# huggingface/parler-tts

Hardware: NVIDIA H100
Metric: audio codec tokens/sec (all codebooks) (higher is better)
Workload: dtype bf16

## Files before the change

### parler_tts_b200/csrc/api.cu

```cuda
#include <cstdarg>
#include <cstdlib>
#include <cstring>
#include <new>
#include <vector>

#include "common.cuh"
#include "dac.h"
#include "kernels.h"
#include "layout.h"
#include "step.h"

namespace ptts {
static thread_local std::string g_err;
void set_error(const std::string& m) { g_err = m; }
int fail(int code, const char* fmt, ...) {
  char buf[1024];
  va_list ap;
  va_start(ap, fmt);
  vsnprintf(buf, sizeof(buf), fmt, ap);
  va_end(ap);
  g_err = buf;
  return code;
}
static bool env_flag(const char* name, bool dflt) {
// ... 4 lines not shown
}

using namespace ptts;

enum DecodePath {
  DECODE_MULTI_KERNEL = 0,
  DECODE_STEP = 1,
  DECODE_CLUSTER = 2,
};

struct ProbeWindow {
  void* self_attn; void* cross_attn; void* hidden;
  int first_step, n_steps;
  int64_t self_ld, self_step, cross_step, hidden_step;
};

struct AlignWindow {
  const int32_t* heads; int n_heads;
  std::vector<int> layer_heads;
  int key0, key_len;
  float* out;
  int first_row, n_rows;
};

struct ptts_session {
  ptts_decoder_config cfg;
  DecoderLayout L;
  WorkspaceLayout W;
  const char* blob;
  char* ws;
  int sm_count;
  bool has_prompt_mask, has_enc_mask, begun, prefilled;
  ptts_gen_params gen;
  int n0;
  bool ragged;
  int sampled;
  bool decoded;
  bool slots;
  cudaStream_t cap_stream;
  cudaGraphExec_t exec;
  bool graph_ready;
  int64_t launches;
  long long* prof;
  DecodePath path;
  StepParams sp;
  ptts_sampling_ext ext;
  ptts_logits_ext lext;
  SampleOut out;
  ProbeWindow probe;
  AlignWindow align;
  int64_t graph_launches;
};

static const ptts_sampling_ext kExtOff = {0, 0.f, 1.f, 0.f, 0.f};
static const ptts_sampling_ext* active_ext(const ptts_session* s) {
  const ptts_sampling_ext& x = s->ext;
  const bool warp = s->gen.do_sample && (x.min_p > 0.f || x.typical_p < 1.f || x.epsilon_cutoff > 0.f || x.eta_cutoff > 0.f);
  return (x.no_repeat_ngram_size > 0 || warp) ? &s->ext : nullptr;
}
static const ptts_logits_ext* active_lext(const ptts_session* s) {
  const ptts_logits_ext& x = s->lext;
  const bool on = x.bias1 != nullptr || x.n_seq > 0 || x.forced_bos_token_id >= 0 || x.forced_eos_token_id >= 0 ||
                  x.remove_invalid_values || x.decay != nullptr || x.suppress != nullptr || x.begin_suppress != nullptr ||
                  x.renormalize_logits;
  return on ? &s->lext : nullptr;
}
static const SampleOut* active_out(const ptts_session* s) {
  return (s->out.logits != nullptr || s->out.scores != nullptr) ? &s->out : nullptr;
}
static const ProbeWindow* active_probe(const ptts_session* s) {
  const ProbeWindow& w = s->probe;
  return (w.self_attn != nullptr || w.cross_attn != nullptr || w.hidden != nullptr) ? &w : nullptr;
}
static const AlignWindow* active_align(const ptts_session* s) { return s->align.out != nullptr ? &s->align : nullptr; }
static DecodePath decode_path(const ptts_session* s) {
  return (active_probe(s) != nullptr || active_align(s) != nullptr) ? DECODE_MULTI_KERNEL : s->path;
}

static const ptts_sampling_ext* sampler_ext(const ptts_session* s) {
  const ptts_sampling_ext* x = active_ext(s);
  return (x == nullptr && (active_out(s) != nullptr || active_lext(s) != nullptr || s->slots)) ? &kExtOff : x;
}
static const int* slot_keys(const ptts_session* s) { return s->slots ? (const int*)(s->ws + s->W.row_key) : nullptr; }

extern "C" {

const char* ptts_last_error(void) { return g_err.c_str(); }
int ptts_version(void) { return 100; }

int ptts_decoder_blob_bytes(const ptts_decoder_config* cfg, int64_t* out_bytes) {
  PTTS_REQUIRE(cfg && out_bytes, "null argument");
  if (int e = validate_config(*cfg)) return e;
  *out_bytes = make_layout(*cfg).total;
  return PTTS_OK;
}

int ptts_decoder_pack(const ptts_decoder_config* cfg, void* blob, int32_t tensor_id, int32_t index, const void* src,
                      int32_t src_dtype, int64_t rows, int64_t cols, void* stream) {
  PTTS_REQUIRE(cfg && blob && src, "null argument");
  if (int e = validate_config(*cfg)) return e;
  PTTS_REQUIRE(src_dtype == PTTS_BF16 || src_dtype == PTTS_F32, "pack: src dtype must be bf16 or f32");
  const DecoderLayout L = make_layout(*cfg);
  cudaStream_t st = (cudaStream_t)stream;
  char* base = (char*)blob;
  MatSlot ms;
  const bool per_layer = (tensor_id >= PTTS_T_LN1_W && tensor_id <= PTTS_T_FC2);
  if (per_layer) PTTS_REQUIRE(index >= 0 && index < L.L, "pack: layer %d out of range", index);
  if (matrix_slot(L, tensor_id, index, &ms)) {
    if (tensor_id == PTTS_T_LM_HEAD) PTTS_REQUIRE(index >= 0 && index < L.K, "pack: codebook %d out of range", index);
    PTTS_REQUIRE(cols == ms.m.K, "pack: tensor %d expects %d columns, got %lld", tensor_id, ms.m.K, (long long)cols);
    PTTS_REQUIRE(rows > 0 && ms.row_off + rows <= ms.m.N, "pack: tensor %d rows %lld do not fit fused matrix of %d rows", tensor_id, (long long)rows, ms.m.N);
    return pack_matrix(src, src_dtype, rows, cols, ms.row_off, ms.m.K, base + ms.m.w, cfg->dtype, st);
  }
  const int H = L.H;
  switch (tensor_id) {
    case PTTS_T_EMBED_TOKENS:
      PTTS_REQUIRE(index >= 0 && index < L.K && rows == L.V + 1 && cols == H, "pack: embed_tokens shape");
      return pack_plain(src, src_dtype, rows * cols, base + L.embed + (int64_t)index * (L.V + 1) * H * L.es, cfg->dtype, st);
    case PTTS_T_POS_TABLE:
      PTTS_REQUIRE(!cfg->rope && rows == cfg->max_positions && cols == H, "pack: pos table shape");
      return pack_plain(src, src_dtype, rows * cols, base + L.pos, cfg->dtype, st);
    case PTTS_T_ROPE_COS:
    case PTTS_T_ROPE_SIN:
      PTTS_REQUIRE(cfg->rope && rows == cfg->max_positions && cols == PTTS_HEAD_DIM, "pack: rope table shape");
      return pack_plain(src, src_dtype, rows * cols, base + (tensor_id == PTTS_T_ROPE_COS ? L.rope_cos : L.rope_sin), cfg->dtype, st);
    case PTTS_T_LN1_W: case PTTS_T_LN1_B: case PTTS_T_LN2_W: case PTTS_T_LN2_B: case PTTS_T_LN3_W: case PTTS_T_LN3_B:
    case PTTS_T_FINAL_LN_W: case PTTS_T_FINAL_LN_B: {
      PTTS_REQUIRE(rows * cols == H, "pack: LayerNorm parameter must have %d elements", H);
      const int m = tensor_id <= PTTS_T_LN1_B ? MAT_QKV : tensor_id <= PTTS_T_LN2_B ? MAT_Q_CROSS : tensor_id <= PTTS_T_LN3_B ? MAT_FC1 : MAT_HEADS;
      const DecoderMatrix dm = decoder_matrix(L, m, index);
      const bool gamma = tensor_id == PTTS_T_LN1_W || tensor_id == PTTS_T_LN2_W || tensor_id == PTTS_T_LN3_W || tensor_id == PTTS_T_FINAL_LN_W;
      return pack_plain(src, src_dtype, H, base + (gamma ? dm.ln_w : dm.ln_b), PTTS_F32, st);
    }
    default:
      return fail(PTTS_EINVAL, "pack: unknown tensor id %d", tensor_id);
  }
}

int ptts_decoder_finalize(const ptts_decoder_config* cfg, void* blob, void* stream) {
  PTTS_REQUIRE(cfg && blob, "null argument");
  if (int e = validate_config(*cfg)) return e;
  if (cfg->dtype != PTTS_BF16) return PTTS_OK;
  const DecoderLayout L = make_layout(*cfg);
  cudaStream_t st = (cudaStream_t)stream;
  char* b = (char*)blob;
  for (int m = 0; m < MAT_COUNT; m++)
    for (int i = 0; i < (m == MAT_HEADS ? 1 : L.L); i++) {
      const DecoderMatrix d = decoder_matrix(L, m, i);
      if (d.ln_w >= 0) {
        float* c = (float*)(b + d.c);
        if (int e = fold_layernorm(b + d.w, d.N, d.K, (const float*)(b + d.ln_w), (const float*)(b + d.ln_b), c, c + d.N, st)) return e;
      }
      if (d.rm >= 0)
        if (int e = unpack_fragments(b + d.w, b + d.rm, d.N, d.K, st)) return e;
    }
  if (L.cl_NC > 0) {
    for (int i = 0; i < L.L; i++)
      if (int e = cluster_pack_layer(L, b + L.layer0 + L.layer_stride * i, st)) return e;
  }
  return PTTS_OK;
}

int ptts_workspace_bytes3(const ptts_decoder_config* cfg, int32_t B, int32_t P, int32_t S, int32_t max_cache_len, int32_t max_input_len,
                          int32_t takes, int64_t* out_bytes) {
  PTTS_REQUIRE(cfg && out_bytes, "null argument");
  if (int e = validate_config(*cfg)) return e;
// ... 501 lines not shown
  const WorkspaceLayout& W = s->W;
  PTTS_REQUIRE(T >= 1 && T <= W.max_input, "score: %d decoder input columns, the session takes 1 .. %d", T, W.max_input);
  PTTS_REQUIRE(W.P == 0 || prompt_hidden, "score: prompt_hidden is required when P > 0");
  PTTS_REQUIRE(labels ? (out_token_nll != nullptr) : (out_logits != nullptr && out_codebook_sums == nullptr),
               "score: labels need out_token_nll; without labels only out_logits can be filled");
  const bool fused = (c.dtype == PTTS_BF16 && out_logits == nullptr);
  PTTS_REQUIRE(!fused || heads_rm, "score: the fused bf16 path needs the row-major heads (ptts_lm_heads_rowmajor_pack)");
  PTTS_REQUIRE(!fused || score_fused_supported(L.H, L.V), "score: hidden_size %d / vocab_size %d are outside the fused kernel", L.H, L.V);
  cudaStream_t st = (cudaStream_t)stream;
  PTTS_CHECK_CUDA(cudaMemcpy2DAsync(s->ws + W.raw_ids, W.raw_ld * 8, dec_ids, (size_t)T * 8, (size_t)T * 8, W.BK, cudaMemcpyDeviceToDevice, st));
  s->has_prompt_mask = (prompt_mask != nullptr && W.P > 0);
  s->has_enc_mask = (enc_mask != nullptr);
  if (s->has_prompt_mask) { if (int e = launch_mask_convert(prompt_mask, W.B * W.P, (int*)(s->ws + W.prompt_mask), st)) return e; }
  if (s->has_enc_mask) { if (int e = launch_mask_convert(enc_mask, W.B / W.takes * W.S, (int*)(s->ws + W.enc_mask), st)) return e; }
  s->n0 = T;
  s->ragged = s->slots = false;
  s->begun = s->prefilled = false;
  if (int e = run_forward(s, st, true, prompt_hidden, enc_hidden, false)) return e;

  ScoreArgs a{};
  a.labels = labels; a.dec_ids = dec_ids; a.token_nll = out_token_nll;
  a.M = W.B * T; a.B = W.B; a.T = T; a.K = L.K; a.V = L.V; a.H = L.H;
  a.bos = c.bos_token_id; a.eos = c.eos_token_id;
  const int q_len = W.P + T;
  const DecoderMatrix hm = decoder_matrix(L, MAT_HEADS, 0);
  if (fused) {
    a.c1 = (const float*)(s->blob + hm.c); a.c2 = a.c1 + hm.N;
    s->launches += 2;
    if (int e = launch_score_fused(a, s->ws + W.x, W.P, c.layer_norm_eps, s->ws + W.qc, (float*)(s->ws + W.row_stats), heads_rm, st)) return e;
  } else {
    for (int t = 0; t < T; t++) {
      LinearArgs h{};
      h.X = s->ws + W.x + (int64_t)(W.P + t) * L.H * L.es; h.ldx = (int64_t)q_len * L.H;
      h.W = s->blob + hm.w; h.Y = s->ws + W.logits; h.ldy = hm.N; h.ldr = h.ldy;
      h.ln_w = (const float*)(s->blob + hm.ln_w); h.ln_b = (const float*)(s->blob + hm.ln_b); h.eps = c.layer_norm_eps;
      if (c.dtype == PTTS_BF16) { h.c1 = (const float*)(s->blob + hm.c); h.c2 = h.c1 + hm.N; }
      h.M = W.B; h.N = hm.N; h.K = hm.K; h.Kc = hm.K;
      h.epi = EPI_F32; h.act = c.activation;
      if (int e = launch_linear(h, c.dtype, st, false, s->sm_count)) return e;
      if (int e = launch_score_rows(a, (const float*)(s->ws + W.logits), t, out_logits, st)) return e;
      s->launches += 2;
    }
  }
  if (out_codebook_sums != nullptr) {
    s->launches++;
    if (int e = launch_score_reduce(a, out_codebook_sums, st)) return e;
  }
  return PTTS_OK;
}

int ptts_decode_forward(ptts_session* s, void* stream) {
  PTTS_REQUIRE(s, "null argument");
  if (!s->prefilled) return fail(PTTS_ESTATE, "ptts_decode_forward called before ptts_prefill");
  cudaStream_t st = (cudaStream_t)stream;
  s->decoded = true;
  StepParams p = s->sp;
  p.do_sample_phase = 0;
  switch (decode_path(s)) {
    case DECODE_CLUSTER: s->launches++; return launch_decode_step_cluster(p, st);
    case DECODE_STEP: s->launches++; return launch_decode_step(p, s->sm_count, st);
    case DECODE_MULTI_KERNEL: break;
  }
  return run_forward(s, st, false, nullptr, nullptr);
}

int ptts_sample(ptts_session* s, const int64_t* forced_tokens, void* stream) {
  PTTS_REQUIRE(s, "null argument");
  if (!s->prefilled) return fail(PTTS_ESTATE, "ptts_sample called before ptts_prefill");
  s->launches++;
  s->sampled++;
  return launch_sample(sample_args(s), forced_tokens, (cudaStream_t)stream, false, sampler_ext(s), active_out(s), active_lext(s),
                       slot_keys(s));
}

int ptts_decode_steps(ptts_session* s, int32_t n_steps, void* stream) {
  PTTS_REQUIRE(s && n_steps >= 0, "bad argument");
  if (!s->prefilled) return fail(PTTS_ESTATE, "ptts_decode_steps called before ptts_prefill");
  cudaStream_t st = (cudaStream_t)stream;
  if (n_steps > 0) s->decoded = true;
  const ptts_sampling_ext* ext = sampler_ext(s);
  const SampleOut* out = active_out(s);
  const ptts_logits_ext* lext = active_lext(s);
  const DecodePath path = decode_path(s);
  if (ext != nullptr && path != DECODE_MULTI_KERNEL) {
    StepParams p = s->sp;
    p.do_sample_phase = 0;
    for (int i = 0; i < n_steps; i++) {
      const int e = path == DECODE_CLUSTER ? launch_decode_step_cluster(p, st) : launch_decode_step(p, s->sm_count, st);
      if (e) return e;
      if (int e2 = launch_sample(sample_args(s), nullptr, st, false, ext, out, lext, slot_keys(s))) return e2;
    }
    s->launches += 2 * (int64_t)n_steps;
    return PTTS_OK;
  }
  switch (path) {
    case DECODE_CLUSTER: {
      const char* env = getenv("PTTS_STEPS_PER_LAUNCH");
      const int per_launch = env ? (atoi(env) < 1 ? 1 : atoi(env)) : 64;
      for (int done = 0; done < n_steps;) {
        const int m = (n_steps - done < per_launch) ? n_steps - done : per_launch;
        s->sp.n_steps = m;
        const int e = launch_decode_step_cluster(s->sp, st);
        s->sp.n_steps = 1;
        if (e) return e;
        done += m;
        s->launches += 1;
      }
      return PTTS_OK;
    }
    case DECODE_STEP:
      for (int i = 0; i < n_steps; i++)
        if (int e = launch_decode_step(s->sp, s->sm_count, st)) return e;
      s->launches += n_steps;
      return PTTS_OK;
    case DECODE_MULTI_KERNEL: break;
  }
  if (!s->graph_ready) {
    if (!s->cap_stream) PTTS_CHECK_CUDA(cudaStreamCreateWithFlags(&s->cap_stream, cudaStreamNonBlocking));
    const int64_t before = s->launches;
    PTTS_CHECK_CUDA(cudaStreamBeginCapture(s->cap_stream, cudaStreamCaptureModeThreadLocal));
    int e = run_forward(s, s->cap_stream, false, nullptr, nullptr);
    if (!e) { s->launches++; e = launch_sample(sample_args(s), nullptr, s->cap_stream, true, ext, out, lext, slot_keys(s)); }
    cudaGraph_t graph = nullptr;
    cudaError_t ce = cudaStreamEndCapture(s->cap_stream, &graph);
    s->graph_launches = s->launches - before;
    s->launches = before;
    if (e) { if (graph) cudaGraphDestroy(graph); return e; }
    if (ce != cudaSuccess) return fail(PTTS_ECUDA, "graph capture failed: %s", cudaGetErrorString(ce));
    ce = cudaGraphInstantiate(&s->exec, graph, 0);
    cudaGraphDestroy(graph);
    if (ce != cudaSuccess) return fail(PTTS_ECUDA, "graph instantiate failed: %s", cudaGetErrorString(ce));
    s->graph_ready = true;
  }
  for (int i = 0; i < n_steps; i++) PTTS_CHECK_CUDA(cudaGraphLaunch(s->exec, st));
  s->launches += s->graph_launches * n_steps;
  return PTTS_OK;
}

int ptts_session_import_rows(ptts_session* dst, const ptts_session* src, const int32_t* src_rows, const int32_t* dst_rows, int32_t n,
                             void* stream) {
  PTTS_REQUIRE(dst && src && (n == 0 || (src_rows && dst_rows)) && n >= 0, "bad argument");
  if (!src->prefilled || !dst->prefilled) return fail(PTTS_ESTATE, "import_rows: both sessions must have run ptts_prefill");
  PTTS_REQUIRE(dst != src, "import_rows: the source and the destination are one session");
  PTTS_REQUIRE(memcmp(&src->cfg, &dst->cfg, sizeof(src->cfg)) == 0 && src->blob == dst->blob, "import_rows: the sessions run different models");
  PTTS_REQUIRE(src->W.P == dst->W.P && src->W.S == dst->W.S, "import_rows: P and S must match (source %d, %d; destination %d, %d)",
               src->W.P, src->W.S, dst->W.P, dst->W.S);
  PTTS_REQUIRE(src->W.takes == 1 && dst->W.takes == 1, "import_rows: sessions with takes > 1 share cross K/V between rows");
  PTTS_REQUIRE(src->has_prompt_mask == dst->has_prompt_mask && src->has_enc_mask == dst->has_enc_mask,
               "import_rows: both sessions must have been prefilled with the same masks given (or both without)");
  PTTS_REQUIRE(!src->ragged && src->n0 == 1, "import_rows: the source rows must start from the BOS column (a uniform generation)");
  PTTS_REQUIRE(src->sampled == 1 && !src->decoded, "import_rows: the source must have run ptts_prefill and exactly one ptts_sample "
               "since (%d samples%s)", src->sampled, src->decoded ? " and decode steps" : "");
  const int kv_len = src->W.P + src->n0;
  PTTS_REQUIRE(kv_len <= dst->W.Tmax, "import_rows: %d cache positions do not fit the destination's %d", kv_len, dst->W.Tmax);
  RowImportArgs a{};
  RowRegion tmp[kMaxRowRegions];
  a.n_regions = row_regions(src->cfg, src->W, kv_len, a.src);
  PTTS_REQUIRE(row_regions(dst->cfg, dst->W, kv_len, tmp) == a.n_regions, "import_rows: the sessions hold different per-row state "
               "(create both with the same max_input_len class: 1, or >= 2)");
  for (int r = 0; r < a.n_regions; r++) a.dst[r] = tmp[r];
  a.src_ws = src->ws; a.dst_ws = dst->ws; a.K = src->cfg.num_codebooks;
  a.src_ctrl = (const Ctrl*)(src->ws + src->W.ctrl); a.dst_ctrl = (const Ctrl*)(dst->ws + dst->W.ctrl);
  std::vector<char> taken(dst->W.B, 0);
  for (int i = 0; i < n; i++) {
    PTTS_REQUIRE(src_rows[i] >= 0 && src_rows[i] < src->W.B, "import_rows: source row %d outside [0, %d)", src_rows[i], src->W.B);
    PTTS_REQUIRE(dst_rows[i] >= 0 && dst_rows[i] < dst->W.B, "import_rows: destination row %d outside [0, %d)", dst_rows[i], dst->W.B);
    PTTS_REQUIRE(!taken[dst_rows[i]], "import_rows: destination row %d is listed twice", dst_rows[i]);
    taken[dst_rows[i]] = 1;
  }
  for (int i0 = 0; i0 < n; i0 += kMaxImportRows) {
    const int m = n - i0 < kMaxImportRows ? n - i0 : kMaxImportRows;
    for (int i = 0; i < m; i++) { a.src_row[i] = src_rows[i0 + i]; a.dst_row[i] = dst_rows[i0 + i]; }
    if (int e = launch_import_rows(a, m, (cudaStream_t)stream)) return e;
// ... 297 lines not shown
```

### parler_tts_b200/csrc/step.h

```cpp
#pragma once
#include "common.cuh"
#include "kernels.h"
#include "layout.h"

namespace ptts {

struct StepParams {
  int B, H, F, V, K, L, nh, nkv, nckv, S, P, Tmax, rope, act, qkv_rows, ckv_rows;
  int takes;
  float eps, scale;
  const char* blob;
  DecoderLayout lay;
  bf16 *x, *qkv, *attn, *qc, *hbuf;
  float* logits;
  char* cross_kv; int64_t cross_layer_stride;
  char* self_kv; int64_t self_layer_stride;
  const int* prompt_mask;
  const int* enc_mask;
  SampleArgs sa;
  unsigned* bar;
  int nt_qkv, nt_h, nt_fc1, nt_heads;
  int nbuf;
  int64_t tile_region_bytes;
  int64_t wbuf_offset;
  int do_sample_phase;
  int sample_items;
  int* progress;
  int n_steps;
  long long* prof;
  bf16 *cl_x, *cl_attn, *cl_h;
};

const char* plan_decode_step(StepParams& p, int grid);
int launch_decode_step(const StepParams& p, int grid, cudaStream_t st);
bool cluster_step_available(const StepParams& p);
int launch_decode_step_cluster(const StepParams& p, cudaStream_t st);
int cluster_pack_layer(const DecoderLayout& L, char* layer, cudaStream_t st);

}
```

### parler_tts_b200/csrc/step2.cu

```cuda
#include "attn_core.cuh"
#include "common.cuh"
#include "kernels.h"
#include "ln_stats.cuh"
#include "sample_core.cuh"
#include "ptx.cuh"
#include "step.h"
#include "step_common.cuh"
#include <type_traits>

namespace ptts {
namespace cl {

constexpr int C = 2;
constexpr int V = 8;
constexpr int THREADS = 256;
constexpr int ROWS = 32;
constexpr int HROWS = 8;
constexpr int ATT_SMEM = attn_decode_smem_per_warp<bf16>();
constexpr int PROF_STRIDE = 16;
constexpr int QMAX = 6;
constexpr int OFF_STATS = 256, OFF_PART = 512, OFF_RES = 2560, OFF_CVEC = 3584;
constexpr int HDR = 5632;
constexpr int WB_BYTES = 65536;
constexpr int R_OFF = HDR + 2 * WB_BYTES;
// ... 25 lines not shown
  asm volatile("st.async.shared::cluster.mbarrier::complete_tx::bytes.b32 [%0], %1, [%2];"
               ::"r"(dst_cluster_addr), "r"(__float_as_uint(v)), "r"(bar_cluster_addr) : "memory");
}
__device__ __forceinline__ void st_async(uint32_t dst_cluster_addr, float2 v, uint32_t bar_cluster_addr) {
  asm volatile("st.async.shared::cluster.mbarrier::complete_tx::bytes.v2.f32 [%0], {%1, %2}, [%3];"
               ::"r"(dst_cluster_addr), "f"(v.x), "f"(v.y), "r"(bar_cluster_addr) : "memory");
}
__device__ __forceinline__ uint32_t mapa(uint32_t addr, uint32_t rank) { uint32_t r; asm volatile("mapa.shared::cluster.u32 %0, %1, %2;" : "=r"(r) : "r"(addr), "r"(rank)); return r; }
__device__ __forceinline__ uint32_t cluster_rank() { uint32_t r; asm volatile("mov.u32 %0, %%cluster_ctarank;" : "=r"(r)); return r; }
__device__ __forceinline__ void cluster_arrive() { asm volatile("barrier.cluster.arrive.release.aligned;" ::: "memory"); }
__device__ __forceinline__ void cluster_wait() { asm volatile("barrier.cluster.wait.acquire.aligned;" ::: "memory"); }
__device__ __forceinline__ void cluster_arrive_reuse() { asm volatile("barrier.cluster.arrive.relaxed.aligned;" ::: "memory"); }

__host__ __device__ __forceinline__ int kslice(int kt) { return (kt & 7) >> 2; }
__host__ __device__ __forceinline__ int klocal(int kt) { return ((kt >> 3) << 2) | (kt & 3); }
__host__ __device__ __forceinline__ int kglobal(int rank, int lk) { return ((lk >> 2) << 3) | (rank << 2) | (lk & 3); }

template <int QN, int MT, bool STATS, bool ACC = false>
__device__ __forceinline__ void mma_slice(float (&out)[2][6][4], RowStatFrag& rst, const bf16* xs, int apitch, const uint4* wb, int KT, int kt0,
                                          int kt_end, int lrow, int lcol) {
  float acc[MT][QN][4];
#pragma unroll
  for (int a = 0; a < MT; a++)
#pragma unroll
    for (int j = 0; j < QN; j++)
#pragma unroll
      for (int e = 0; e < 4; e++) acc[a][j][e] = ACC ? out[a][j][e] : 0.f;
  for (int kt = kt0; kt < kt_end; kt += 4) {
    uint32_t a[MT][2][4];
#pragma unroll
    for (int mt = 0; mt < MT; mt++)
#pragma unroll
      for (int j = 0; j < 2; j++) ldmatrix_x4(a[mt][j], xs + (size_t)(mt * 16 + lrow) * apitch + kt * 32 + j * 16 + lcol);
    if (STATS) {
#pragma unroll
      for (int mt = 0; mt < MT; mt++) { row_stat_mma(rst, mt, a[mt][0]); row_stat_mma(rst, mt, a[mt][1]); }
    }
#pragma unroll
    for (int j = 0; j < QN; j++) {
      const uint4 w = wb[((size_t)j * KT + kt) * 32];
#pragma unroll
      for (int mt = 0; mt < MT; mt++) {
        mma_bf16_16816(acc[mt][j], a[mt][0], w.x, w.y);
        mma_bf16_16816(acc[mt][j], a[mt][1], w.z, w.w);
      }
    }
  }
#pragma unroll
  for (int mt = 0; mt < MT; mt++)
#pragma unroll
    for (int j = 0; j < QN; j++)
#pragma unroll
      for (int e = 0; e < 4; e++) out[mt][j][e] = acc[mt][j][e];
}

enum { PH_QKV = 0, PH_O = 1, PH_QC = 2, PH_OC = 3, PH_FC1 = 4, PH_FC2 = 5 };
constexpr int JOBS_PER_LAYER = 9;
constexpr int QKV_JOBS = 4;

__device__ __forceinline__ bool weight_job(const StepParams& p, int j, int cta, int rank, const char*& src, uint32_t& bytes) {
  const int nl = JOBS_PER_LAYER * p.L;
  if (j < nl) {
    const int l = j / JOBS_PER_LAYER, jl = j - JOBS_PER_LAYER * l;
    const int ph = jl < QKV_JOBS ? 0 : jl - (QKV_JOBS - 1);
    const int64_t idx = (ph == PH_QKV || ph == PH_QC) ? (int64_t)(cta >> 3) * C + rank : (int64_t)cta;
    const int64_t sz = p.lay.cp_slice[ph];
    bytes = (uint32_t)(ph == PH_QKV ? sz / QKV_JOBS : sz);
    src = p.blob + p.lay.layer0 + p.lay.layer_stride * l + p.lay.cp[ph] + idx * sz + (ph == PH_QKV ? jl * (sz / QKV_JOBS) : 0);
    return true;
  }
  const int task = cta + (int)gridDim.x * (j - nl);
  const int ntasks = p.K * p.V / 32;
  if (task >= ntasks) return false;
  bytes = (uint32_t)(4 * p.H * 16);
  src = p.blob + p.lay.heads + (int64_t)task * bytes;
  return true;
}

template <int ITEMS, bool RAGGED>
__global__ void __launch_bounds__(THREADS, 1) decode_step_cluster_kernel(const __grid_constant__ StepParams p) {
  extern __shared__ __align__(128) unsigned char smem[];
  Ctrl* ctrl = p.sa.ctrl;
  if (p.prof != nullptr && blockIdx.x == 0 && threadIdx.x == 0) p.prof[(size_t)(6 * p.L + 2) * PROF_STRIDE + 3] = clock64();
  if (ctrl->active == 0) return;
  int cur_len = ctrl->cur_len;
  const unsigned gen = (unsigned)ctrl->launch_gen;
  int pos = p.P + cur_len - 1;
  const int tid = threadIdx.x, warp = tid >> 5, lane = tid & 31;
  const int H = p.H, F = p.F, B = p.B;
  const int rank = (int)cluster_rank(), peer = rank ^ 1;
  const int cta = (int)blockIdx.x;
  const int cluster = cta >> 1;
  const int head = cluster >> 2, rblk = cluster & 3;
  const int Ks = H / C, KsF = F / 4;
  const int pitch = Ks + 8, pitchF = KsF + 8;
  const int qe = F / p.nh / 64;
  const int dgrp = warp & 1, e4 = warp >> 1;

  uint64_t* abar = reinterpret_cast<uint64_t*>(smem);
  uint64_t* wbar = abar + 1;
  uint64_t* xbar = abar + 3;
  uint64_t* attbars = reinterpret_cast<uint64_t*>(smem + 128);
  float* stats = reinterpret_cast<float*>(smem + OFF_STATS);
  float* part = reinterpret_cast<float*>(smem + OFF_PART);
  float* res_s = reinterpret_cast<float*>(smem + OFF_RES);
  float* cvec = reinterpret_cast<float*>(smem + OFF_CVEC);
  unsigned char* Rg = smem + R_OFF;
  const uint32_t peer_xbar = mapa(smem_u32(xbar), (uint32_t)peer);
  uint32_t par_a = 0, par_w = 0, par_x = 0, att_parity = 0;

  if (tid == 0) {
    mbar_init<1>(abar); mbar_init<1>(&wbar[0]); mbar_init<1>(&wbar[1]); mbar_init<1>(xbar);
    asm volatile("fence.mbarrier_init.release.cluster;" ::: "memory");
  }
  attention_decode_init_warp(attbars + 2 * warp, lane);
  cluster_arrive(); cluster_wait();
  unsigned* const bar_ctr = p.bar + (gen & 1u);
  unsigned bar_target = 0u;
  if (cta == 0 && tid == 0) p.bar[(gen + 1u) & 1u] = 0u;

  const char* blob = p.blob;
  long long* const prof0 = (p.prof != nullptr && cta == 0) ? p.prof : nullptr;
  long long* prof = prof0;
  prof_mark(prof, 0);

  auto issue_weight_job = [&](int j) {
    const char* src; uint32_t bytes;
    if (!weight_job(p, j, cta, rank, src, bytes)) return;
    mbar_expect_tx(&wbar[j & 1], bytes);
    bulk_g2s_evict_first(smem + HDR + (j & 1) * WB_BYTES, src, bytes, &wbar[j & 1]);
  };
  __shared__ int s_next_active;
  const int n_steps = (p.do_sample_phase && p.n_steps > 1 && prof0 == nullptr) ? p.n_steps : 1;
  int unfinished_prev = 0;
#pragma unroll 1
  for (int it = 0; it < n_steps; it++) {
  pos = p.P + cur_len - 1;
  prof = prof0;
  cluster_arrive_reuse();
  if (tid == 0) { issue_weight_job(0); issue_weight_job(1); }

  bf16* const x_img = p.cl_x;
  bf16* const a_img = p.cl_attn;
  bf16* const h_img = p.cl_h;
  const int x_slice_elems = ROWS * pitch, h_slice_elems = ROWS * pitchF;
  auto h_offset = [&](int n) {
    const int lk = klocal(n >> 5), kq = KsF >> 5;
    return (size_t)(2 * kslice(n >> 5) + lk / kq) * h_slice_elems + (lk % kq) * 32 + (n & 31);
  };
  const int xo_slice = kslice(cta >> 2), xo_col = klocal(cta >> 2) * 32 + (cta & 3) * 8;

  {
    const int row = tid >> 3, f = tid & 7, n = cta * 8 + f;
    const float v = row < B ? embed_value(p, row, n, row_pos<RAGGED>(p, row, pos)) : 0.f;
    res_s[row * 8 + f] = v;
    x_img[(size_t)xo_slice * x_slice_elems + row * pitch + xo_col + f] = __float2bfloat16_rn(v);
  }
  prof_mark(prof, 6);
  auto request_slice = [&](const bf16* img_slice, uint32_t bytes) {
    fence_proxy_async_smem();
    mbar_expect_tx(abar, bytes);
    bulk_g2s(Rg, img_slice, bytes, abar);
  };
  auto slice_of = [&](int sub, const bf16*& img, uint32_t& bytes) {
    if (sub == PH_QKV || sub == PH_QC) { img = x_img + (size_t)rank * x_slice_elems + (size_t)(HROWS * rblk) * pitch; bytes = (uint32_t)(HROWS * pitch * 2); }
    else if (sub == PH_O || sub == PH_OC) { img = a_img + (size_t)rank * x_slice_elems; bytes = (uint32_t)(x_slice_elems * 2); }
    else if (sub == PH_FC1) { img = x_img + (size_t)rank * x_slice_elems; bytes = (uint32_t)(x_slice_elems * 2); }
    else { img = h_img + (size_t)(2 * rank) * h_slice_elems; bytes = (uint32_t)(h_slice_elems * 2); }
  };
  {
    const bf16* nimg; uint32_t nbytes;
    slice_of(PH_QKV, nimg, nbytes);
    bar_target = grid_sync(bar_ctr, bar_target, -1, false, nullptr, [&]() { request_slice(nimg, nbytes); });
  }
  prof_mark(prof, 7);

  const int lrow = (lane & 7) + ((lane >> 3) & 1) * 8, lcol = (lane >> 4) * 8;
  const int g = lane >> 2, t4 = lane & 3;
  const int n_phases = 6 * p.L;

  const int att_row = HROWS * rblk + 4 * rank + (warp >> 1);
  const int att_slice = kslice(2 * head), att_col = klocal(2 * head) * 32;

#pragma unroll 1
  for (int ph = 0; ph < n_phases; ph++) {
    const int l = ph / 6, sub = ph - 6 * l;
    prof = prof0 ? prof0 + (size_t)(ph + 1) * PROF_STRIDE : nullptr;
    prof_mark(prof, 0);
    const char* lb = blob + p.lay.layer0 + p.lay.layer_stride * l;
    const bool rowpart = (sub == PH_QKV || sub == PH_QC);
    const bool has_ln = (sub == PH_QKV || sub == PH_QC || sub == PH_FC1);
    const int q = (sub == PH_QKV) ? 6 : (sub == PH_QC ? 2 : (sub == PH_FC1 ? qe : 1));
    const int Nc = 4 * q * 8;
    const int KT = (sub == PH_FC2 ? KsF : Ks) >> 5;
    const int apitch = (sub == PH_FC2) ? pitchF : pitch;
    const int act_bytes = (rowpart ? HROWS : ROWS) * apitch * 2;
    const int RS = (q == 1) ? 8 : 8 * q + 2;
    const int blk = rowpart ? 32 + 4 * 16 * q * 4 : 256 + ROWS * RS * 4;
    unsigned char* const recv = Rg + ((act_bytes + 127) & ~127);
    const uint32_t peer_recv = mapa(smem_u32(recv), (uint32_t)peer);
    const uint32_t xbytes = 4u * (rowpart ? V * 4 * 16 * q + V / 2 * 4 * 2 : V / C * (ROWS * 8 * q + (has_ln ? ROWS * 2 : 0)));
    auto put = [&](int d, uint32_t off, auto v) {
      if (d == rank) *reinterpret_cast<decltype(v)*>(recv + off) = v;
      else st_async(peer_recv + off, v, peer_xbar);
    };
    const int j0 = JOBS_PER_LAYER * l + (sub == 0 ? 0 : sub + QKV_JOBS - 1);
    if (tid == 0) mbar_expect_tx(xbar, xbytes);

    auto att_stage0 = [&]() -> unsigned char* {
      if (sub == PH_QC) return Rg + ATT_S0_QC + warp * ATT_STAGE;
      return warp < 6 ? Rg + ATT_S0_QKV + warp * ATT_STAGE : smem + HDR + (warp - 6) * WB_BYTES + ATT_S0_WB;
    };
    if (rowpart && att_row < B)
      attention_decode_request<bf16>(decode_attn_args(p, l, pos, sub == PH_QC), att_row, head, row_pos<RAGGED>(p, att_row, pos), att_stage0(),
                                     attbars + 2 * warp, lane, warp & 1, 2);

    float cv1 = 0.f, cv2 = 0.f;
    if (has_ln) {
      const float* c1; int ntot;
      if (sub == PH_QKV) { c1 = reinterpret_cast<const float*>(lb + p.lay.c_qkv); ntot = p.qkv_rows; }
      else if (sub == PH_QC) { c1 = reinterpret_cast<const float*>(lb + p.lay.c_qc); ntot = H; }
      else { c1 = reinterpret_cast<const float*>(lb + p.lay.c_fc1); ntot = F; }
      const int nown = rowpart ? Nc : 8 * q;
// ... 241 lines not shown
      RowStatFrag rst;
      row_stat_zero(rst);
      for (int kt = warp; kt < KTH; kt += 8) {
        const bf16* sl = ktile(kt);
#pragma unroll
        for (int mt = 0; mt < 2; mt++)
#pragma unroll
          for (int j = 0; j < 2; j++) {
            uint32_t a[4];
            ldmatrix_x4(a, sl + (size_t)(mt * 16 + lrow) * pitch + j * 16 + lcol);
            row_stat_mma(rst, mt, a);
          }
      }
      row_stat_store(rst, part, warp, lane);
      __syncthreads();
      row_stat_finalize(part, H, ROWS, p.eps, stats);
      __syncthreads();
    }
    prof_mark(prof, 1);
    constexpr int HRS = 40;
    int job = JOBS_PER_LAYER * p.L;
    for (int task = cta; task < ntasks; task += (int)gridDim.x, job++) {
      mbar_wait(&wbar[job & 1], (par_w >> (job & 1)) & 1u, 4);
      par_w ^= 1u << (job & 1);
      float acc[2][4][4];
#pragma unroll
      for (int a = 0; a < 2; a++)
#pragma unroll
        for (int j = 0; j < 4; j++)
#pragma unroll
          for (int e = 0; e < 4; e++) acc[a][j][e] = 0.f;
      unsigned char* wbuf = smem + HDR + (job & 1) * WB_BYTES;
      const uint4* wb = reinterpret_cast<const uint4*>(wbuf) + lane;
      for (int kt = warp; kt < KTH; kt += 8) {
        const bf16* sl = ktile(kt);
        uint32_t a[2][2][4];
#pragma unroll
        for (int mt = 0; mt < 2; mt++)
#pragma unroll
          for (int j = 0; j < 2; j++) ldmatrix_x4(a[mt][j], sl + (size_t)(mt * 16 + lrow) * pitch + j * 16 + lcol);
#pragma unroll
        for (int j = 0; j < 4; j++) {
          const uint4 w = wb[((size_t)j * KTH + kt) * 32];
#pragma unroll
          for (int mt = 0; mt < 2; mt++) {
            mma_bf16_16816(acc[mt][j], a[mt][0], w.x, w.y);
            mma_bf16_16816(acc[mt][j], a[mt][1], w.z, w.w);
          }
        }
      }
      __syncthreads();
      float* red = reinterpret_cast<float*>(wbuf);
#pragma unroll
      for (int mt = 0; mt < 2; mt++)
#pragma unroll
        for (int j = 0; j < 4; j++) {
          float* base = red + ((size_t)warp * 32 + mt * 16 + g) * HRS + j * 8 + 2 * t4;
          *reinterpret_cast<float2*>(base) = make_float2(acc[mt][j][0], acc[mt][j][1]);
          *reinterpret_cast<float2*>(base + 8 * HRS) = make_float2(acc[mt][j][2], acc[mt][j][3]);
        }
      __syncthreads();
      {
        const int er = tid >> 3, ec = tid & 7;
        if (er < B) {
          const float mean = stats[2 * er], rstd = stats[2 * er + 1];
#pragma unroll
          for (int j = 0; j < 4; j++) {
            const int cidx = j * 8 + ec, n = task * 32 + cidx;
            float v = 0.f;
#pragma unroll
            for (int w = 0; w < 8; w++) v += red[((size_t)w * 32 + er) * HRS + cidx];
            p.logits[(size_t)er * p.K * p.V + n] = DT<bf16>::rnd(rstd * (v - mean * c1[n]) + c2[n]);
          }
        }
      }
      __syncthreads();
      if (tid == 32) {
        fence_proxy_async_smem();
        issue_weight_job(job + 2);
      }
    }
  }
  prof_mark(prof, 6);
  bar_target = grid_sync(bar_ctr, bar_target, n_phases, true);
  prof = prof0 ? prof0 + (size_t)(n_phases + 2) * PROF_STRIDE : nullptr;
  prof_mark(prof, 0);
  if (p.do_sample_phase) {
    const ptts_gen_params gp = *p.sa.gen;
    const int BK = B * p.K;
    sample_phase<ITEMS, RAGGED>(p.sa, gp, BK, cur_len);
    prof_mark(prof, 1);
    bar_target = grid_sync(bar_ctr, bar_target, n_phases + 1, true, nullptr, [&]() {
      const int tot = *reinterpret_cast<volatile int*>(&ctrl->n_unfinished);
      s_next_active = (tot - unfinished_prev > 0) ? 1 : 0;
      unfinished_prev = tot;
    });
    prof_mark(prof, 2);
  }
  bool go_on = false;
  if (p.do_sample_phase) {
    const int act = s_next_active;
    if (cta == 0 && tid == 0) {
      ctrl->cur_len = cur_len + 1;
      ctrl->active = act;
      ctrl->steps_run += 1;
    }
    go_on = act != 0;
    cur_len += 1;
  }
  if (!go_on) break;
  }
  if (cta == 0 && tid == 0) {
    if (p.do_sample_phase) ctrl->n_unfinished = 0;
    ctrl->launch_gen = (int)(gen + 1u);
  }
}

__global__ void cluster_pack_kernel(const uint4* __restrict__ src, uint4* __restrict__ dst, int ph, int nh, int ntc, int kts, int KT_src) {
  const int64_t tile = blockIdx.x;
  const int ktl = (int)(tile % kts);
  const int j = (int)((tile / kts) % ntc);
  const int slice = (int)(tile / ((int64_t)kts * ntc));
  const int rank = slice & 1, owner = slice >> 1;
  int n_tile;
  if (ph == PH_QKV) n_tile = (j >> 3) * (nh * 8) + owner * 8 + (j & 7);
  else n_tile = owner * ntc + j;
  const int kt = kglobal(rank, ktl);
  dst[tile * 32 + threadIdx.x] = src[((int64_t)n_tile * KT_src + kt) * 32 + threadIdx.x];
}

}

int cluster_pack_layer(const DecoderLayout& L, char* layer, cudaStream_t st) {
  for (int ph = 0; ph < 6; ph++) {
    const ClusterPhase cp = cluster_phase(L, ph);
    const int64_t tiles = (int64_t)cp.owners * cl::C * cp.nt * cp.kt;
    cl::cluster_pack_kernel<<<(unsigned)tiles, 32, 0, st>>>(reinterpret_cast<const uint4*>(layer + cp.mat),
                                                            reinterpret_cast<uint4*>(layer + L.cp[ph]), ph, L.nh, cp.nt, cp.kt, cp.kt_src);
  }
  PTTS_LAUNCH_CHECK();
  return PTTS_OK;
}

static const void* cluster_kernel_fn(const StepParams& p) {
  const bool rg = p.sa.shift != nullptr;
  if (p.sample_items <= 1) return rg ? (const void*)cl::decode_step_cluster_kernel<1, true> : (const void*)cl::decode_step_cluster_kernel<1, false>;
  if (p.sample_items <= 5) return rg ? (const void*)cl::decode_step_cluster_kernel<5, true> : (const void*)cl::decode_step_cluster_kernel<5, false>;
  return rg ? (const void*)cl::decode_step_cluster_kernel<9, true> : (const void*)cl::decode_step_cluster_kernel<9, false>;
}

static void cluster_launch_config(const StepParams& p, cudaLaunchConfig_t& cfg, cudaLaunchAttribute* at, cudaStream_t st) {
  cfg = cudaLaunchConfig_t{};
  cfg.gridDim = dim3((unsigned)(4 * p.nh * cl::C));
  cfg.blockDim = dim3(cl::THREADS);
  cfg.dynamicSmemBytes = cl::SMEM_BYTES;
  cfg.stream = st;
  at[0].id = cudaLaunchAttributeClusterDimension;
  at[0].val.clusterDim.x = cl::C; at[0].val.clusterDim.y = 1; at[0].val.clusterDim.z = 1;
  at[1].id = cudaLaunchAttributeCooperative;
  at[1].val.cooperative = 1;
  cfg.attrs = at;
  cfg.numAttrs = 2;
}

bool cluster_step_available(const StepParams& p) {
  const void* fn = cluster_kernel_fn(p);
  static bool told = false;
  auto why = [&](const char* what, cudaError_t e, int n) {
    if (!told) fprintf(stderr, "ptts_b200: cluster step kernel not used (%s: %s, %d co-resident clusters of %d, need %d); the one-CTA-per-SM step kernel runs instead\n",
                       what, cudaGetErrorString(e), n, cl::C, 4 * p.nh);
    told = true;
    cudaGetLastError();
    return false;
  };
  cudaError_t e = cudaFuncSetAttribute(fn, cudaFuncAttributeMaxDynamicSharedMemorySize, cl::SMEM_BYTES);
  if (e != cudaSuccess) return why("shared memory attribute", e, 0);
  cudaLaunchConfig_t cfg; cudaLaunchAttribute at[2];
  cluster_launch_config(p, cfg, at, nullptr);
  cfg.numAttrs = 1;
  int n = 0;
  e = cudaOccupancyMaxActiveClusters(&n, fn, &cfg);
  if (e != cudaSuccess) return why("cluster occupancy query", e, n);
  if (n < 4 * p.nh) return why("too few co-resident clusters", cudaSuccess, n);
  return true;
}

int launch_decode_step_cluster(const StepParams& p, cudaStream_t st) {
  const void* fn = cluster_kernel_fn(p);
  cudaLaunchConfig_t cfg; cudaLaunchAttribute at[2];
  cluster_launch_config(p, cfg, at, st);
  void* args[] = {(void*)&p};
  PTTS_CHECK_CUDA(cudaLaunchKernelExC(&cfg, fn, args));
  return PTTS_OK;
}

}
```

Before: 255,900.

## Split cluster decode into step+sample launches with programmatic dependent launch overlap

Result: no change. 255,900, median of 6 (+0.0%).

```diff
diff --git a/parler_tts_b200/csrc/api.cu b/parler_tts_b200/csrc/api.cu
--- a/parler_tts_b200/csrc/api.cu
+++ b/parler_tts_b200/csrc/api.cu
@@ -110,6 +110,12 @@
   return (x == nullptr && (active_out(s) != nullptr || active_lext(s) != nullptr || s->slots)) ? &kExtOff : x;
 }
 static const int* slot_keys(const ptts_session* s) { return s->slots ? (const int*)(s->ws + s->W.row_key) : nullptr; }
+
+static bool cluster_token_loop_persistent(const ptts_session* s) {
+  if (sampler_ext(s) != nullptr) return false;
+  const char* m = getenv("PTTS_TOKEN_LOOP");
+  return !(m != nullptr && strcmp(m, "split") == 0);
+}
 
 extern "C" {
 
@@ -777,13 +783,14 @@
   const SampleOut* out = active_out(s);
   const ptts_logits_ext* lext = active_lext(s);
   const DecodePath path = decode_path(s);
-  if (ext != nullptr && path != DECODE_MULTI_KERNEL) {
+  if ((path == DECODE_CLUSTER && !cluster_token_loop_persistent(s)) || (path == DECODE_STEP && ext != nullptr)) {
     StepParams p = s->sp;
     p.do_sample_phase = 0;
+    const bool pdl = path == DECODE_CLUSTER && env_flag("PTTS_PDL", true);
     for (int i = 0; i < n_steps; i++) {
-      const int e = path == DECODE_CLUSTER ? launch_decode_step_cluster(p, st) : launch_decode_step(p, s->sm_count, st);
+      const int e = path == DECODE_CLUSTER ? launch_decode_step_cluster(p, st, pdl) : launch_decode_step(p, s->sm_count, st);
       if (e) return e;
-      if (int e2 = launch_sample(sample_args(s), nullptr, st, false, ext, out, lext, slot_keys(s))) return e2;
+      if (int e2 = launch_sample(sample_args(s), nullptr, st, pdl, ext, out, lext, slot_keys(s))) return e2;
     }
     s->launches += 2 * (int64_t)n_steps;
     return PTTS_OK;
diff --git a/parler_tts_b200/csrc/step.h b/parler_tts_b200/csrc/step.h
--- a/parler_tts_b200/csrc/step.h
+++ b/parler_tts_b200/csrc/step.h
@@ -34,7 +34,7 @@
 const char* plan_decode_step(StepParams& p, int grid);
 int launch_decode_step(const StepParams& p, int grid, cudaStream_t st);
 bool cluster_step_available(const StepParams& p);
-int launch_decode_step_cluster(const StepParams& p, cudaStream_t st);
+int launch_decode_step_cluster(const StepParams& p, cudaStream_t st, bool pdl = false);
 int cluster_pack_layer(const DecoderLayout& L, char* layer, cudaStream_t st);
 
 }
diff --git a/parler_tts_b200/csrc/step2.cu b/parler_tts_b200/csrc/step2.cu
--- a/parler_tts_b200/csrc/step2.cu
+++ b/parler_tts_b200/csrc/step2.cu
@@ -131,10 +131,6 @@
   extern __shared__ __align__(128) unsigned char smem[];
   Ctrl* ctrl = p.sa.ctrl;
   if (p.prof != nullptr && blockIdx.x == 0 && threadIdx.x == 0) p.prof[(size_t)(6 * p.L + 2) * PROF_STRIDE + 3] = clock64();
-  if (ctrl->active == 0) return;
-  int cur_len = ctrl->cur_len;
-  const unsigned gen = (unsigned)ctrl->launch_gen;
-  int pos = p.P + cur_len - 1;
   const int tid = threadIdx.x, warp = tid >> 5, lane = tid & 31;
   const int H = p.H, F = p.F, B = p.B;
   const int rank = (int)cluster_rank(), peer = rank ^ 1;
@@ -164,14 +160,6 @@
   }
   attention_decode_init_warp(attbars + 2 * warp, lane);
   cluster_arrive(); cluster_wait();
-  unsigned* const bar_ctr = p.bar + (gen & 1u);
-  unsigned bar_target = 0u;
-  if (cta == 0 && tid == 0) p.bar[(gen + 1u) & 1u] = 0u;
-
-  const char* blob = p.blob;
-  long long* const prof0 = (p.prof != nullptr && cta == 0) ? p.prof : nullptr;
-  long long* prof = prof0;
-  prof_mark(prof, 0);
 
   auto issue_weight_job = [&](int j) {
     const char* src; uint32_t bytes;
@@ -179,6 +167,23 @@
     mbar_expect_tx(&wbar[j & 1], bytes);
     bulk_g2s_evict_first(smem + HDR + (j & 1) * WB_BYTES, src, bytes, &wbar[j & 1]);
   };
+  if (tid == 0) { issue_weight_job(0); issue_weight_job(1); }
+  pdl_wait();
+  if (ctrl->active == 0) {
+    if (tid == 0) { mbar_wait(&wbar[0], 0u, 1); mbar_wait(&wbar[1], 0u, 1); }
+    return;
+  }
+  int cur_len = ctrl->cur_len;
+  const unsigned gen = (unsigned)ctrl->launch_gen;
+  int pos = p.P + cur_len - 1;
+  unsigned* const bar_ctr = p.bar + (gen & 1u);
+  unsigned bar_target = 0u;
+  if (cta == 0 && tid == 0) p.bar[(gen + 1u) & 1u] = 0u;
+
+  const char* blob = p.blob;
+  long long* const prof0 = (p.prof != nullptr && cta == 0) ? p.prof : nullptr;
+  long long* prof = prof0;
+  prof_mark(prof, 0);
   __shared__ int s_next_active;
   const int n_steps = (p.do_sample_phase && p.n_steps > 1 && prof0 == nullptr) ? p.n_steps : 1;
   int unfinished_prev = 0;
@@ -187,7 +192,7 @@
   pos = p.P + cur_len - 1;
   prof = prof0;
   cluster_arrive_reuse();
-  if (tid == 0) { issue_weight_job(0); issue_weight_job(1); }
+  if (tid == 0 && it > 0) { issue_weight_job(0); issue_weight_job(1); }
 
   bf16* const x_img = p.cl_x;
   bf16* const a_img = p.cl_attn;
@@ -595,7 +600,8 @@
     }
   }
   prof_mark(prof, 6);
-  bar_target = grid_sync(bar_ctr, bar_target, n_phases, true);
+  if (!p.do_sample_phase) pdl_launch_dependents();
+  else bar_target = grid_sync(bar_ctr, bar_target, n_phases, true);
   prof = prof0 ? prof0 + (size_t)(n_phases + 2) * PROF_STRIDE : nullptr;
   prof_mark(prof, 0);
   if (p.do_sample_phase) {
@@ -662,7 +668,7 @@
   return rg ? (const void*)cl::decode_step_cluster_kernel<9, true> : (const void*)cl::decode_step_cluster_kernel<9, false>;
 }
 
-static void cluster_launch_config(const StepParams& p, cudaLaunchConfig_t& cfg, cudaLaunchAttribute* at, cudaStream_t st) {
+static void cluster_launch_config(const StepParams& p, cudaLaunchConfig_t& cfg, cudaLaunchAttribute* at, cudaStream_t st, bool pdl = false) {
   cfg = cudaLaunchConfig_t{};
   cfg.gridDim = dim3((unsigned)(4 * p.nh * cl::C));
   cfg.blockDim = dim3(cl::THREADS);
@@ -672,8 +678,10 @@
   at[0].val.clusterDim.x = cl::C; at[0].val.clusterDim.y = 1; at[0].val.clusterDim.z = 1;
   at[1].id = cudaLaunchAttributeCooperative;
   at[1].val.cooperative = 1;
+  at[2].id = cudaLaunchAttributeProgrammaticStreamSerialization;
+  at[2].val.programmaticStreamSerializationAllowed = 1;
   cfg.attrs = at;
-  cfg.numAttrs = 2;
+  cfg.numAttrs = pdl ? 3 : 2;
 }
 
 bool cluster_step_available(const StepParams& p) {
@@ -688,7 +696,7 @@
   };
   cudaError_t e = cudaFuncSetAttribute(fn, cudaFuncAttributeMaxDynamicSharedMemorySize, cl::SMEM_BYTES);
   if (e != cudaSuccess) return why("shared memory attribute", e, 0);
-  cudaLaunchConfig_t cfg; cudaLaunchAttribute at[2];
+  cudaLaunchConfig_t cfg; cudaLaunchAttribute at[3];
   cluster_launch_config(p, cfg, at, nullptr);
   cfg.numAttrs = 1;
   int n = 0;
@@ -698,11 +706,21 @@
   return true;
 }
 
-int launch_decode_step_cluster(const StepParams& p, cudaStream_t st) {
+int launch_decode_step_cluster(const StepParams& p, cudaStream_t st, bool pdl) {
   const void* fn = cluster_kernel_fn(p);
-  cudaLaunchConfig_t cfg; cudaLaunchAttribute at[2];
+  cudaLaunchConfig_t cfg; cudaLaunchAttribute at[3];
+  void* args[] = {(void*)&p};
+  static bool pdl_refused = false;
+  if (pdl && !pdl_refused) {
+    cluster_launch_config(p, cfg, at, st, true);
+    const cudaError_t e = cudaLaunchKernelExC(&cfg, fn, args);
+    if (e == cudaSuccess) return PTTS_OK;
+    cudaGetLastError();
+    pdl_refused = true;
+    fprintf(stderr, "ptts_b200: programmatic dependent launch of the cluster step kernel refused (%s: %s); plain launches instead\n",
+            cudaGetErrorName(e), cudaGetErrorString(e));
+  }
   cluster_launch_config(p, cfg, at, st);
-  void* args[] = {(void*)&p};
   PTTS_CHECK_CUDA(cudaLaunchKernelExC(&cfg, fn, args));
   return PTTS_OK;
 }
```
